# achinastone/Tensorium

Hardware: AMD Instinct MI355X
Metric: fp32 SGEMM GFLOP/s (M=N=K=4096) + YOLOv3 conv-fwd images/s (higher is better)
Workload: dtype fp32; 1 GPU; sgemm_nn_4096x4096x4096; M=4096, N=4096, K=4096, parallelism=1 independent replicas, one process per GPU, no data-path collective

## Files before the change

### tensorium_amd/csrc/conv_slab.hip

```cpp
#include <algorithm>
#include <type_traits>

#include "tns_act.hpp"
#include "tns_internal.hpp"

namespace tns {
namespace {

typedef float floatx4 __attribute__((ext_vector_type(4)));

__device__ __forceinline__ void slab_dma16(const float* sbase, unsigned voff, unsigned lds) {
  unsigned keep;
  asm volatile(
      "s_mov_b32 %0, m0\n\ts_mov_b32 m0, %3\n\ts_nop 0\n\t"
      "global_load_lds_dwordx4 %1, %2\n\ts_mov_b32 m0, %0"
      : "=&s"(keep)
      : "v"(voff), "s"(sbase), "s"(lds)
      : "memory");
}

struct SlabFillArgs {
  const float* x;
  int64_t strideX;
  float* slab;
  int C, H, W, stride, pad, dil, ow, ohw, N, K, KT;
  float inv_ohw, inv_ow;
  unsigned bytes;
  int64_t units;
};

__device__ __forceinline__ int slab_div(int n, int d, float inv) {
  int qq = (int)((float)n * inv);
  while (qq * d > n) --qq;
  while ((qq + 1) * d <= n) ++qq;
  return qq;
}

template <int KS, int BK, int BN>
__global__ __launch_bounds__(256) void slab_fill_kernel(SlabFillArgs a) {
  constexpr int NG = BK / 16, KK = KS * KS;
  const int64_t x = (int64_t)blockIdx.x * 256 + threadIdx.x;
  if (x >= a.units) return;
  const int c = (int)(x % BN);
  const int64_t r1 = x / BN;
  const int g = (int)(r1 % NG);
  const int64_t r2 = r1 / NG;
  const int t = (int)(r2 % a.KT), ct = (int)(r2 / a.KT);
  const int n = ct * BN + c;
  float v[16];
  const __amdgpu_buffer_rsrc_t rsrc =
      __builtin_amdgcn_make_buffer_rsrc(const_cast<float*>(a.x), 0, a.bytes, 0x00020000);
  {
    const int nn = n < a.N ? n : a.N - 1;
    const int img = slab_div(nn, a.ohw, a.inv_ohw), pix = nn - img * a.ohw;
    const int oy = slab_div(pix, a.ow, a.inv_ow), ox = pix - oy * a.ow;
    const int iy0 = oy * a.stride - a.pad, ix0 = ox * a.stride - a.pad;
    const int HW = a.H * a.W;
    unsigned mask = 0;
    int toff[KK];
#pragma unroll
    for (int kr = 0; kr < KS; ++kr)
#pragma unroll
      for (int kc = 0; kc < KS; ++kc) {
        const int iy = iy0 + kr * a.dil, ix = ix0 + kc * a.dil;
        mask |= (unsigned)(((unsigned)iy < (unsigned)a.H) & ((unsigned)ix < (unsigned)a.W))
                << (kr * KS + kc);
        toff[kr * KS + kc] = 4 * (kr * a.dil * a.W + kc * a.dil);
      }
    if (n >= a.N) mask = 0;
    const unsigned base = 4u * (unsigned)(img * (int)a.strideX + iy0 * a.W + ix0);
    const int k0 = t * BK + 16 * g;
    int ch = k0 / KK, tap = k0 - ch * KK;
#pragma unroll
    for (int e = 0; e < 16; ++e) {
      int off = toff[0];
#pragma unroll
      for (int u = 1; u < KK; ++u) off = tap == u ? toff[u] : off;
      const unsigned o = ((mask >> tap) & 1u) ? base + 4u * (unsigned)(ch * HW) + (unsigned)off
                                              : 0x80000000u;
      v[e] = __builtin_bit_cast(float, __builtin_amdgcn_raw_buffer_load_b32(rsrc, o, 0, 0));
      if (++tap == KK) {
        tap = 0;
        ++ch;
      }
    }
  }
  float* dst = a.slab + ((r2 * NG + g) * 4 * BN + c) * 4;
#pragma unroll
  for (int q = 0; q < 4; ++q)
    *reinterpret_cast<floatx4*>(dst + q * BN * 4) = floatx4{v[q], v[4 + q], v[8 + q], v[12 + q]};
}

template <int KS, int BK, int BN>
__global__ __launch_bounds__((BN + 63) / 64 * 64) void slab_fill_u_kernel(SlabFillArgs a) {
  constexpr int NG = BK / 16, KK = KS * KS;
  const int c = threadIdx.x;
  if (c >= BN) return;
  const int64_t r1 = blockIdx.x;
  const int g = (int)(r1 % NG);
  const int64_t r2 = r1 / NG;
  const int t = (int)(r2 % a.KT), ct = (int)(r2 / a.KT);
  const int n = ct * BN + c;
  float v[16];
  const __amdgpu_buffer_rsrc_t rsrc =
      __builtin_amdgcn_make_buffer_rsrc(const_cast<float*>(a.x), 0, a.bytes, 0x00020000);
  {
    const int nn = n < a.N ? n : a.N - 1;
    const int img = slab_div(nn, a.ohw, a.inv_ohw), pix = nn - img * a.ohw;
    const int oy = slab_div(pix, a.ow, a.inv_ow), ox = pix - oy * a.ow;
    const int iy0 = oy * a.stride - a.pad, ix0 = ox * a.stride - a.pad;
    const int HW = a.H * a.W;
    unsigned mask = 0;
#pragma unroll
    for (int kr = 0; kr < KS; ++kr)
#pragma unroll
      for (int kc = 0; kc < KS; ++kc) {
        const int iy = iy0 + kr * a.dil, ix = ix0 + kc * a.dil;
        mask |= (unsigned)(((unsigned)iy < (unsigned)a.H) & ((unsigned)ix < (unsigned)a.W))
                << (kr * KS + kc);
      }
    if (n >= a.N) mask = 0;
    const unsigned base = 4u * (unsigned)(img * (int)a.strideX + iy0 * a.W + ix0);
    const int k0 = __builtin_amdgcn_readfirstlane(t * BK + 16 * g);
    int ch = k0 / KK, tap = k0 - ch * KK;
    int kr = tap / KS, kc = tap - kr * KS;
#pragma unroll
    for (int e = 0; e < 16; ++e) {
      const unsigned uoff = 4u * (unsigned)(ch * HW + kr * a.dil * a.W + kc * a.dil);
      const unsigned o = ((mask >> tap) & 1u) ? base + uoff : 0x80000000u;
      v[e] = __builtin_bit_cast(float, __builtin_amdgcn_raw_buffer_load_b32(rsrc, o, 0, 0));
      ++tap;
      if (++kc == KS) {
        kc = 0;
        ++kr;
      }
      if (tap == KK) {
        tap = 0;
        kr = 0;
        ++ch;
      }
    }
  }
  float* dst = a.slab + ((r2 * NG + g) * 4 * BN + c) * 4;
#pragma unroll
  for (int q = 0; q < 4; ++q)
    *reinterpret_cast<floatx4*>(dst + q * BN * 4) = floatx4{v[q], v[4 + q], v[8 + q], v[12 + q]};
}

struct SlabGemmArgs {
  const float* A;
  const float* slab;
  float* C;
  const float* bias;
  int M, N, K, KT, tiles_m, ohw, act;
  bool fuse;
};

template <int BM_, int BN_, int BK_, int WM_, int WN_, int JA_, int NA_, int NS_, int DG_ = 0,
          int MAP_ = 0>
struct SG {
  static constexpr int BM = BM_, BN = BN_, BK = BK_, WM = WM_, WN = WN_, JA = JA_, NA = NA_;
  static constexpr int NS = NS_;
  static constexpr int DG = DG_, MAP = MAP_;
  static constexpr int NW = WM * WN, NT = 64 * NW, J = BN / 16, NG = BK / 16, ROWS = BK / 4;
  static constexpr int JB = NA < WN ? (J - NA * JA) / (WN - NA) : 0;
  static constexpr int A_TILE = ROWS * BM * 4, B_TILE = ROWS * BN * 4, STAGE = A_TILE + B_TILE;
  static constexpr int AU = BM * BK / 4 / NT;
  static constexpr int BDMA = 4 * BK * BN / 1024;
  static constexpr int DPW = (BDMA + NW - 1) / NW;
  static_assert(BM == 16 * WM && BN % 16 == 0 && BK % 16 == 0, "geometry");
  static_assert(NA * JA + (WN - NA) * JB == J && NA >= 1 && NA <= WN, "wave column split");
  static_assert(AU >= 1 && BM * BK / 4 % NT == 0, "A units");
  static_assert(4 * BK * BN % 1024 == 0, "whole DMA instructions");
  static_assert(NS >= 2 && NS * STAGE * 4 <= 163840, "LDS");
  static_assert(NG >= 2 && NG % 2 == 0, "groups: f0 holds group 0 at every tile start");
  static_assert(DPW * (NS - 2) <= 63 && DPW <= 63, "vmcnt immediates");
};

template <int JW>
struct SFrag {
  floatx4 a, b[JW];
};

template <int N>
__device__ __forceinline__ void wait_vm(bool keep_n) {
  if (keep_n)
    asm volatile("s_waitcnt vmcnt(%0)" ::"n"(N) : "memory");
  else
    asm volatile("s_waitcnt vmcnt(0)" ::: "memory");
}

template <class G>
__global__ __launch_bounds__(G::NT, 1) void slab_gemm_kernel(SlabGemmArgs p) {
  constexpr int BM = G::BM, BN = G::BN, BK = G::BK, NG = G::NG, NS = G::NS;
  constexpr int A_TILE = G::A_TILE, STAGE = G::STAGE, AU = G::AU, DPW = G::DPW;
  __shared__ __attribute__((aligned(16))) float smem[NS * STAGE];
  const int tid = threadIdx.x, lane = tid & 63;
  const int w = __builtin_amdgcn_readfirstlane(tid >> 6), wm = w % G::WM, wn = w / G::WM;
  const int r16 = lane & 15, q = lane >> 4;
  int tm, tn;
  {
    const int nb = gridDim.x, bid = blockIdx.x;
    const int xcd = bid & 7, qq = nb >> 3, rr = nb & 7;
    const int wg = (xcd < rr ? xcd * (qq + 1) : rr * (qq + 1) + (xcd - rr) * qq) + (bid >> 3);
    if constexpr (G::MAP == 1) {
      const int tiles_n = (p.N + BN - 1) / BN;
      tn = wg % tiles_n;
      tm = wg / tiles_n;
    } else {
      tm = wg % p.tiles_m;
      tn = wg / p.tiles_m;
    }
  }
  const int m0 = tm * BM, n0 = tn * BN;
  const int N = p.N, K = p.K, nt = p.KT;
  const float* slabT = p.slab + (int64_t)tn * K * BN;
  const unsigned lds0 = (unsigned)(uintptr_t)(__attribute__((address_space(3))) float*)smem;
  const unsigned voff = 16u * (unsigned)lane;
  auto dma_b = [&](int t, int st, int v) {
    if constexpr (G::DG & 1) return;
    int u = w + G::NW * v;
    if (G::BDMA % G::NW != 0 && u >= G::BDMA) u -= G::NW;
    slab_dma16(slabT + (int64_t)t * (BK * BN) + 256 * u, voff,
               lds0 + 4u * (unsigned)(st * STAGE + A_TILE) + 1024u * (unsigned)u);
  };
  auto dma_all = [&](int t, int st) {
#pragma unroll
    for (int v = 0; v < DPW; ++v) dma_b(t, st, v);
  };
  unsigned a_off[AU];
  int a_dst[AU];
#pragma unroll
  for (int u = 0; u < AU; ++u) {
    const int idx = tid + G::NT * u;
    const int lo = idx & 7, rest = idx >> 3;
    const int m = rest % BM, kq4 = lo + 8 * (rest / BM);
    a_off[u] = 4u * (unsigned)(m * K + 4 * kq4);
    a_dst[u] = (4 * (kq4 >> 2)) * BM * 4 + m * 4 + (kq4 & 3);
  }
  const float* a_row0 = p.A + (int64_t)m0 * K;
  floatx4 ra[AU];
  auto load_a = [&](int t) {
    if constexpr (G::DG & 2) return;
    const float* sb = a_row0 + t * BK;
#pragma unroll
    for (int u = 0; u < AU; ++u)
      asm volatile("global_load_dwordx4 %0, %1, %2" : "=v"(ra[u]) : "v"(a_off[u]), "s"(sb) : "memory");
  };
  auto store_a = [&](int st) {
    if constexpr (G::DG & 2) return;
    float* as = smem + st * STAGE;
#pragma unroll
    for (int u = 0; u < AU; ++u) {
      asm volatile("" : "+v"(ra[u]));
      as[a_dst[u]] = ra[u][0];
      as[a_dst[u] + BM * 4] = ra[u][1];
      as[a_dst[u] + 2 * BM * 4] = ra[u][2];
      as[a_dst[u] + 3 * BM * 4] = ra[u][3];
    }
  };

  auto run = [&](auto JWC, const int coff) {
    constexpr int JW = decltype(JWC)::value;
    floatx4 acc[JW];
#pragma unroll
    for (int j = 0; j < JW; ++j) acc[j] = floatx4{0.f, 0.f, 0.f, 0.f};
    using Frag = SFrag<JW>;
    auto frag = [&](int st, int g, Frag& f) {
      const float* ap = smem + st * STAGE + ((4 * g + q) * BM + wm * 16 + r16) * 4;
      f.a = *reinterpret_cast<const floatx4*>(ap);
      const float* bp = smem + st * STAGE + A_TILE + ((4 * g + q) * BN + coff * 16 + r16) * 4;
#pragma unroll
      for (int j = 0; j < JW; ++j) f.b[j] = *reinterpret_cast<const floatx4*>(bp + 64 * j);
    };
    auto mma = [&](const Frag& f) {
#pragma unroll
      for (int i = 0; i < 4; ++i)
#pragma unroll
        for (int j = 0; j < JW; ++j)
          acc[j] = __builtin_amdgcn_mfma_f32_16x16x4f32(f.a[i], f.b[j][i], acc[j], 0, 0, 0);
    };
    auto mma_dma = [&](const Frag& f, int tb, int st) {
      constexpr int NM = 4 * JW, STEP = NM / DPW > 0 ? NM / DPW : 1;
#pragma unroll
      for (int x = 0; x < NM; ++x) {
        const int i = x / JW, j = x % JW;
        acc[j] = __builtin_amdgcn_mfma_f32_16x16x4f32(f.a[i], f.b[j][i], acc[j], 0, 0, 0);
        if (x % STEP == 0 && x / STEP < DPW) dma_b(tb, st, x / STEP);
        __builtin_amdgcn_sched_barrier(0);
      }
      if constexpr (NM / STEP < DPW) {
#pragma unroll
        for (int v = NM / STEP; v < DPW; ++v) dma_b(tb, st, v);
      }
    };

    Frag f0, f1;
    load_a(0);
#pragma unroll
    for (int t = 0; t < NS; ++t) {
      if (t == 1 && nt > 1) {
        wait_vm<0>(false);
        store_a(0);
        load_a(1);
      }
      if (t < nt) dma_all(t, t);
    }
    if (nt == 1) {
      wait_vm<0>(false);
      store_a(0);
    } else {
      if (nt >= NS)
        asm volatile("s_waitcnt vmcnt(%0)" ::"n"(AU + (NS - 1) * DPW) : "memory");
      else
        wait_vm<0>(false);
    }
    __syncthreads();
    frag(0, 0, f0);
    for (int t = 0; t < nt; ++t) {
      const int cur = t % NS;
#pragma unroll
      for (int g = 0; g + 1 < NG; ++g) {
        Frag& fc = (g & 1) ? f1 : f0;
        Frag& fn = (g & 1) ? f0 : f1;
        frag(cur, g + 1, fn);
        __builtin_amdgcn_sched_barrier(0);
        mma(fc);
        __builtin_amdgcn_sched_barrier(0);
      }
      if (t + 1 < nt) {
        const int nxt = (t + 1) % NS;
        if constexpr (NS == 2)
          wait_vm<0>(false);
        else
          wait_vm<DPW>(t + NS - 1 < nt);
        store_a(nxt);
        if constexpr (!(G::DG & 4))
          __syncthreads();
        frag(nxt, 0, f0);
        if (t + 2 < nt) load_a(t + 2);
        __builtin_amdgcn_sched_barrier(0);
        if (t + NS < nt)
          mma_dma(f1, t + NS, cur);
        else
          mma(f1);
      } else {
        mma(f1);
      }
    }

    const int row0 = m0 + wm * 16 + 4 * q;
    float bias[4];
#pragma unroll
    for (int e = 0; e < 4; ++e) bias[e] = p.fuse ? p.bias[row0 + e] : 0.0f;
#pragma unroll
    for (int j = 0; j < JW; ++j) {
      const int n = n0 + coff * 16 + 16 * j + r16;
      if (n >= N) continue;
      const int img = n / p.ohw, pix = n - img * p.ohw;
      float* cp = p.C + ((int64_t)img * p.M + row0) * p.ohw + pix;
#pragma unroll
      for (int e = 0; e < 4; ++e) {
        float v = acc[j][e];
        if (p.fuse) v = act_apply_cheap(v + bias[e], p.act);
        cp[(int64_t)e * p.ohw] = v;
      }
    }
  };
  if constexpr (G::NA == G::WN) {
    run(std::integral_constant<int, G::JA>{}, wn * G::JA);
  } else {
    if (wn < G::NA)
      run(std::integral_constant<int, G::JA>{}, wn * G::JA);
    else
      run(std::integral_constant<int, G::JB>{}, G::NA * G::JA + (wn - G::NA) * G::JB);
  }
}

struct SlabForm {
  int bm, bn, bk;
  hipError_t (*gemm)(const SlabGemmArgs&, hipStream_t);
  hipError_t (*fill)(const SlabFillArgs&, int ks, hipStream_t);
  const char* name;
};

template <class G>
hipError_t launch_slab_gemm(const SlabGemmArgs& a, hipStream_t s) {
  const int64_t blocks = (int64_t)(a.M / G::BM) * ((a.N + G::BN - 1) / G::BN);
  hipLaunchKernelGGL((slab_gemm_kernel<G>), dim3((unsigned)blocks), dim3(G::NT), 0, s, a);
  return hipGetLastError();
}

template <int BK, int BN>
hipError_t launch_slab_fill(const SlabFillArgs& a, int ks, hipStream_t s) {
#ifndef TNS_SLAB_FILL_LANE
  {
    constexpr int NT = (BN + 63) / 64 * 64;
    const int64_t nb = a.units / BN;
    if (nb > 0x7fffffffLL) return hipErrorInvalidValue;
    if (ks == 3)
      hipLaunchKernelGGL((slab_fill_u_kernel<3, BK, BN>), dim3((unsigned)nb), dim3(NT), 0, s, a);
    else if (ks == 1)
      hipLaunchKernelGGL((slab_fill_u_kernel<1, BK, BN>), dim3((unsigned)nb), dim3(NT), 0, s, a);
    else
      return hipErrorInvalidValue;
    return hipGetLastError();
  }
#endif
  const unsigned blocks = (unsigned)((a.units + 255) / 256);
  if (ks == 3)
    hipLaunchKernelGGL((slab_fill_kernel<3, BK, BN>), dim3(blocks), dim3(256), 0, s, a);
  else if (ks == 1)
    hipLaunchKernelGGL((slab_fill_kernel<1, BK, BN>), dim3(blocks), dim3(256), 0, s, a);
  else
    return hipErrorInvalidValue;
  return hipGetLastError();
}

#define TNS_SLAB(BMv, BNv, BKv, WMv, WNv, JAv, NAv, NSv)                                       \
  {BMv, BNv, BKv, launch_slab_gemm<SG<BMv, BNv, BKv, WMv, WNv, JAv, NAv, NSv>>,                   \
   launch_slab_fill<BKv, BNv>,                                                                   \
   "conv_slab<" #BMv "x" #BNv "x" #BKv ",w" #WMv "x" #WNv ",j" #JAv "x" #NAv ",s" #NSv ">"}
#define TNS_SLABD(BMv, BNv, BKv, WMv, WNv, JAv, NAv, NSv, DGv, MAPv)                             \
  {BMv, BNv, BKv, launch_slab_gemm<SG<BMv, BNv, BKv, WMv, WNv, JAv, NAv, NSv, DGv, MAPv>>,       \
   launch_slab_fill<BKv, BNv>,                                                                   \
   "conv_slab<" #BMv "x" #BNv "x" #BKv ",w" #WMv "x" #WNv ",j" #JAv "x" #NAv ",s" #NSv ",dg" #DGv \
   ",map" #MAPv ">"}
const SlabForm kSlab[] = {
    TNS_SLAB(32, 176, 64, 2, 4, 3, 3, 3),
    TNS_SLAB(64, 176, 32, 4, 2, 6, 1, 3),
    TNS_SLAB(64, 176, 32, 4, 2, 6, 1, 4),
    TNS_SLAB(32, 176, 64, 2, 4, 3, 3, 2),
    TNS_SLAB(64, 176, 64, 4, 2, 6, 1, 2),
    TNS_SLAB(32, 176, 32, 2, 2, 6, 1, 4),
    TNS_SLABD(32, 176, 64, 2, 4, 3, 3, 2, 0, 1),
    TNS_SLABD(64, 176, 64, 4, 2, 6, 1, 2, 0, 1),
};
#undef TNS_SLAB
#undef TNS_SLABD
constexpr int kNumSlab = sizeof(kSlab) / sizeof(kSlab[0]);

}

int conv_slab_count() { return kNumSlab; }
const char* conv_slab_name(int v) { return v >= 0 && v < kNumSlab ? kSlab[v].name : ""; }

int conv_slab_pick(int64_t M, int64_t N, int64_t K, int64_t ks) {
  if (ks != 3 || K % 64) return -1;
  if (M == 1024 && N >= 1024) return 3;
  if (M == 512 && N >= 4096) return 4;
  return -1;
}

int64_t conv_slab_floats(int v, int64_t N, int64_t K) {
  if (v < 0 || v >= kNumSlab) return -1;
  const int64_t bn = kSlab[v].bn;
  return (N + bn - 1) / bn * bn * K;
}

hipError_t launch_conv_slab(int v, const ConvSlabArgs& c, float* slab, hipStream_t s) {
  if (v < 0 || v >= kNumSlab) return hipErrorInvalidValue;
  const SlabForm& f = kSlab[v];
  const int64_t N = c.batch * c.ohw;
  if (c.M % f.bm || c.K % f.bk || (c.ks != 1 && c.ks != 3) || N >= (1LL << 22) ||
      4 * c.batch * c.C * c.H * c.W > 0x7fffffffLL ||
      c.K > 0x7fffffffLL / f.bn || (reinterpret_cast<uintptr_t>(c.weights) & 15) || c.K % 4 ||
      (reinterpret_cast<uintptr_t>(slab) & 15) || c.M * c.K > 0x7fffffffLL)
    return hipErrorInvalidValue;
  const int64_t CT = (N + f.bn - 1) / f.bn, KT = c.K / f.bk;
  if (CT * (c.M / f.bm) > 0x7fffffffLL) return hipErrorInvalidValue;
  SlabFillArgs fa{};
  fa.x = c.input; fa.strideX = c.C * c.H * c.W; fa.slab = slab;
  fa.C = (int)c.C; fa.H = (int)c.H; fa.W = (int)c.W; fa.stride = (int)c.stride;
  fa.pad = (int)c.pad; fa.dil = (int)c.dil; fa.ow = (int)c.ow; fa.ohw = (int)c.ohw;
  fa.N = (int)N; fa.K = (int)c.K; fa.KT = (int)KT;
  fa.inv_ohw = (float)((1.0 + 1.0 / 1048576.0) / (double)c.ohw);
  fa.inv_ow = (float)((1.0 + 1.0 / 1048576.0) / (double)c.ow);
  fa.bytes = (unsigned)(4 * c.batch * c.C * c.H * c.W);
  fa.units = CT * KT * (f.bk / 16) * f.bn;
  if (hipError_t e = f.fill(fa, (int)c.ks, s)) return e;
  SlabGemmArgs ga{};
  ga.A = c.weights; ga.slab = slab; ga.C = c.out; ga.bias = c.bias;
  ga.M = (int)c.M; ga.N = (int)N; ga.K = (int)c.K; ga.KT = (int)KT;
  ga.tiles_m = (int)(c.M / f.bm); ga.ohw = (int)c.ohw; ga.act = c.act; ga.fuse = c.bias != nullptr;
  return f.gemm(ga, s);
}

}
```

Measured before the change: 148,800 GFLOP/s.

## Deepen A-operand register prefetch in slab conv GEMM pipeline

Adds an A-depth template parameter so the slab GEMM kernel keeps several tiles of A loads in flight in rotating register buffers, and waits with computed vmcnt immediates instead of a single-tile lookahead. The picked variants for the 1024- and 512-channel conv cases now use depths 2 and 4 to hide global-load latency on A with NS=2 LDS stages. It also removes the unused lane-parallel fill kernel. Deeper prefetch costs more VGPRs and a more complex prologue and wait accounting, which risks register pressure or mistimed waits. The SGEMM headline path is not touched.

Measured after the change: 148,800 GFLOP/s. No clear change (-0.0%).

```diff
diff --git a/tensorium_amd/csrc/conv_slab.hip b/tensorium_amd/csrc/conv_slab.hip
--- a/tensorium_amd/csrc/conv_slab.hip
+++ b/tensorium_amd/csrc/conv_slab.hip
@@ -34,61 +34,6 @@
   while (qq * d > n) --qq;
   while ((qq + 1) * d <= n) ++qq;
   return qq;
-}
-
-template <int KS, int BK, int BN>
-__global__ __launch_bounds__(256) void slab_fill_kernel(SlabFillArgs a) {
-  constexpr int NG = BK / 16, KK = KS * KS;
-  const int64_t x = (int64_t)blockIdx.x * 256 + threadIdx.x;
-  if (x >= a.units) return;
-  const int c = (int)(x % BN);
-  const int64_t r1 = x / BN;
-  const int g = (int)(r1 % NG);
-  const int64_t r2 = r1 / NG;
-  const int t = (int)(r2 % a.KT), ct = (int)(r2 / a.KT);
-  const int n = ct * BN + c;
-  float v[16];
-  const __amdgpu_buffer_rsrc_t rsrc =
-      __builtin_amdgcn_make_buffer_rsrc(const_cast<float*>(a.x), 0, a.bytes, 0x00020000);
-  {
-    const int nn = n < a.N ? n : a.N - 1;
-    const int img = slab_div(nn, a.ohw, a.inv_ohw), pix = nn - img * a.ohw;
-    const int oy = slab_div(pix, a.ow, a.inv_ow), ox = pix - oy * a.ow;
-    const int iy0 = oy * a.stride - a.pad, ix0 = ox * a.stride - a.pad;
-    const int HW = a.H * a.W;
-    unsigned mask = 0;
-    int toff[KK];
-#pragma unroll
-    for (int kr = 0; kr < KS; ++kr)
-#pragma unroll
-      for (int kc = 0; kc < KS; ++kc) {
-        const int iy = iy0 + kr * a.dil, ix = ix0 + kc * a.dil;
-        mask |= (unsigned)(((unsigned)iy < (unsigned)a.H) & ((unsigned)ix < (unsigned)a.W))
-                << (kr * KS + kc);
-        toff[kr * KS + kc] = 4 * (kr * a.dil * a.W + kc * a.dil);
-      }
-    if (n >= a.N) mask = 0;
-    const unsigned base = 4u * (unsigned)(img * (int)a.strideX + iy0 * a.W + ix0);
-    const int k0 = t * BK + 16 * g;
-    int ch = k0 / KK, tap = k0 - ch * KK;
-#pragma unroll
-    for (int e = 0; e < 16; ++e) {
-      int off = toff[0];
-#pragma unroll
-      for (int u = 1; u < KK; ++u) off = tap == u ? toff[u] : off;
-      const unsigned o = ((mask >> tap) & 1u) ? base + 4u * (unsigned)(ch * HW) + (unsigned)off
-                                              : 0x80000000u;
-      v[e] = __builtin_bit_cast(float, __builtin_amdgcn_raw_buffer_load_b32(rsrc, o, 0, 0));
-      if (++tap == KK) {
-        tap = 0;
-        ++ch;
-      }
-    }
-  }
-  float* dst = a.slab + ((r2 * NG + g) * 4 * BN + c) * 4;
-#pragma unroll
-  for (int q = 0; q < 4; ++q)
-    *reinterpret_cast<floatx4*>(dst + q * BN * 4) = floatx4{v[q], v[4 + q], v[8 + q], v[12 + q]};
 }
 
 template <int KS, int BK, int BN>
@@ -157,11 +102,12 @@
 };
 
 template <int BM_, int BN_, int BK_, int WM_, int WN_, int JA_, int NA_, int NS_, int DG_ = 0,
-          int MAP_ = 0>
+          int MAP_ = 0, int AD_ = 1>
 struct SG {
   static constexpr int BM = BM_, BN = BN_, BK = BK_, WM = WM_, WN = WN_, JA = JA_, NA = NA_;
   static constexpr int NS = NS_;
   static constexpr int DG = DG_, MAP = MAP_;
+  static constexpr int AD = AD_;
   static constexpr int NW = WM * WN, NT = 64 * NW, J = BN / 16, NG = BK / 16, ROWS = BK / 4;
   static constexpr int JB = NA < WN ? (J - NA * JA) / (WN - NA) : 0;
   static constexpr int A_TILE = ROWS * BM * 4, B_TILE = ROWS * BN * 4, STAGE = A_TILE + B_TILE;
@@ -175,6 +121,10 @@
   static_assert(NS >= 2 && NS * STAGE * 4 <= 163840, "LDS");
   static_assert(NG >= 2 && NG % 2 == 0, "groups: f0 holds group 0 at every tile start");
   static_assert(DPW * (NS - 2) <= 63 && DPW <= 63, "vmcnt immediates");
+  static constexpr int KEEP_A = (AD < NS ? AD : NS) - 1;
+  static constexpr int KEEP_B = AD - 1 < NS - 2 ? AD - 1 : NS - 2;
+  static constexpr int KEEP = AU * KEEP_A + DPW * KEEP_B;
+  static_assert(AD >= 1 && AD <= 4 && (AD == 1 || KEEP <= 63), "A depth");
 };
 
 template <int JW>
@@ -239,24 +189,28 @@
     a_dst[u] = (4 * (kq4 >> 2)) * BM * 4 + m * 4 + (kq4 & 3);
   }
   const float* a_row0 = p.A + (int64_t)m0 * K;
-  floatx4 ra[AU];
-  auto load_a = [&](int t) {
+  constexpr int AD = G::AD;
+  floatx4 ra[AD][AU];
+  auto load_a = [&](int t, floatx4(&r)[AU]) __attribute__((always_inline)) {
     if constexpr (G::DG & 2) return;
     const float* sb = a_row0 + t * BK;
 #pragma unroll
     for (int u = 0; u < AU; ++u)
-      asm volatile("global_load_dwordx4 %0, %1, %2" : "=v"(ra[u]) : "v"(a_off[u]), "s"(sb) : "memory");
+      asm volatile("global_load_dwordx4 %0, %1, %2"
+                   : "=v"(r[u])
+                   : "v"(a_off[u]), "s"(sb)
+                   : "memory");
   };
-  auto store_a = [&](int st) {
+  auto store_a = [&](int st, floatx4(&r)[AU]) __attribute__((always_inline)) {
     if constexpr (G::DG & 2) return;
     float* as = smem + st * STAGE;
 #pragma unroll
     for (int u = 0; u < AU; ++u) {
-      asm volatile("" : "+v"(ra[u]));
-      as[a_dst[u]] = ra[u][0];
-      as[a_dst[u] + BM * 4] = ra[u][1];
-      as[a_dst[u] + 2 * BM * 4] = ra[u][2];
-      as[a_dst[u] + 3 * BM * 4] = ra[u][3];
+      asm volatile("" : "+v"(r[u]));
+      as[a_dst[u]] = r[u][0];
+      as[a_dst[u] + BM * 4] = r[u][1];
+      as[a_dst[u] + 2 * BM * 4] = r[u][2];
+      as[a_dst[u] + 3 * BM * 4] = r[u][3];
     }
   };
 
@@ -296,56 +250,117 @@
     };
 
     Frag f0, f1;
-    load_a(0);
-#pragma unroll
-    for (int t = 0; t < NS; ++t) {
-      if (t == 1 && nt > 1) {
+    if constexpr (AD == 1) {
+      load_a(0, ra[0]);
+#pragma unroll
+      for (int t = 0; t < NS; ++t) {
+        if (t == 1 && nt > 1) {
+          wait_vm<0>(false);
+          store_a(0, ra[0]);
+          load_a(1, ra[0]);
+        }
+        if (t < nt) dma_all(t, t);
+      }
+      if (nt == 1) {
         wait_vm<0>(false);
-        store_a(0);
-        load_a(1);
-      }
-      if (t < nt) dma_all(t, t);
-    }
-    if (nt == 1) {
-      wait_vm<0>(false);
-      store_a(0);
+        store_a(0, ra[0]);
+      } else {
+        if (nt >= NS)
+          asm volatile("s_waitcnt vmcnt(%0)" ::"n"(AU + (NS - 1) * DPW) : "memory");
+        else
+          wait_vm<0>(false);
+      }
+      __syncthreads();
+      frag(0, 0, f0);
+      for (int t = 0; t < nt; ++t) {
+        const int cur = t % NS;
+#pragma unroll
+        for (int g = 0; g + 1 < NG; ++g) {
+          Frag& fc = (g & 1) ? f1 : f0;
+          Frag& fn = (g & 1) ? f0 : f1;
+          frag(cur, g + 1, fn);
+          __builtin_amdgcn_sched_barrier(0);
+          mma(fc);
+          __builtin_amdgcn_sched_barrier(0);
+        }
+        if (t + 1 < nt) {
+          const int nxt = (t + 1) % NS;
+          if constexpr (NS == 2)
+            wait_vm<0>(false);
+          else
+            wait_vm<DPW>(t + NS - 1 < nt);
+          store_a(nxt, ra[0]);
+          if constexpr (!(G::DG & 4))
+            __syncthreads();
+          frag(nxt, 0, f0);
+          if (t + 2 < nt) load_a(t + 2, ra[0]);
+          __builtin_amdgcn_sched_barrier(0);
+          if (t + NS < nt)
+            mma_dma(f1, t + NS, cur);
+          else
+            mma(f1);
+        } else {
+          mma(f1);
+        }
+      }
     } else {
-      if (nt >= NS)
-        asm volatile("s_waitcnt vmcnt(%0)" ::"n"(AU + (NS - 1) * DPW) : "memory");
-      else
-        wait_vm<0>(false);
-    }
-    __syncthreads();
-    frag(0, 0, f0);
-    for (int t = 0; t < nt; ++t) {
-      const int cur = t % NS;
-#pragma unroll
-      for (int g = 0; g + 1 < NG; ++g) {
-        Frag& fc = (g & 1) ? f1 : f0;
-        Frag& fn = (g & 1) ? f0 : f1;
-        frag(cur, g + 1, fn);
-        __builtin_amdgcn_sched_barrier(0);
-        mma(fc);
-        __builtin_amdgcn_sched_barrier(0);
-      }
-      if (t + 1 < nt) {
-        const int nxt = (t + 1) % NS;
-        if constexpr (NS == 2)
-          wait_vm<0>(false);
-        else
-          wait_vm<DPW>(t + NS - 1 < nt);
-        store_a(nxt);
-        if constexpr (!(G::DG & 4))
-          __syncthreads();
-        frag(nxt, 0, f0);
-        if (t + 2 < nt) load_a(t + 2);
-        __builtin_amdgcn_sched_barrier(0);
-        if (t + NS < nt)
-          mma_dma(f1, t + NS, cur);
-        else
+      constexpr int LAG = AD > NS - 1 ? AD : NS - 1;
+      auto slot_dma = [&](int tb) __attribute__((always_inline)) {
+        if (tb >= 0 && tb < nt) dma_all(tb, tb % NS);
+      };
+      constexpr int SL = AD + 1 > NS ? AD + 1 : NS;
+#pragma unroll
+      for (int s = -SL; s <= -2; ++s) {
+        slot_dma(s + NS);
+        const int ta = s + AD + 1;
+        if (ta >= 0 && ta < nt) {
+          if (ta % AD == 0) load_a(ta, ra[0]);
+          if constexpr (AD > 1) if (ta % AD == 1) load_a(ta, ra[1 % AD]);
+          if constexpr (AD > 2) if (ta % AD == 2) load_a(ta, ra[2 % AD]);
+          if constexpr (AD > 3) if (ta % AD == 3) load_a(ta, ra[3 % AD]);
+        }
+      }
+      wait_vm<G::KEEP>(LAG - 1 < nt);
+      store_a(0, ra[0]);
+      __syncthreads();
+      frag(0, 0, f0);
+      slot_dma(NS - 1);
+      if (AD < nt) load_a(AD, ra[0]);
+      auto tile = [&](int t, auto UC) __attribute__((always_inline)) {
+        constexpr int NX = (decltype(UC)::value + 1) % AD;
+        const int cur = t % NS;
+#pragma unroll
+        for (int g = 0; g + 1 < NG; ++g) {
+          Frag& fc = (g & 1) ? f1 : f0;
+          Frag& fn = (g & 1) ? f0 : f1;
+          frag(cur, g + 1, fn);
+          __builtin_amdgcn_sched_barrier(0);
+          mma(fc);
+          __builtin_amdgcn_sched_barrier(0);
+        }
+        if (t + 1 < nt) {
+          const int nxt = (t + 1) % NS;
+          wait_vm<G::KEEP>(t + LAG < nt);
+          store_a(nxt, ra[NX]);
+          if constexpr (!(G::DG & 4))
+            __syncthreads();
+          frag(nxt, 0, f0);
+          __builtin_amdgcn_sched_barrier(0);
+          if (t + NS < nt)
+            mma_dma(f1, t + NS, cur);
+          else
+            mma(f1);
+          __builtin_amdgcn_sched_barrier(0);
+          if (t + AD + 1 < nt) load_a(t + AD + 1, ra[NX]);
+        } else {
           mma(f1);
-      } else {
-        mma(f1);
+        }
+      };
+      for (int t0 = 0; t0 < nt; t0 += AD) {
+        tile(t0, std::integral_constant<int, 0>{});
+        if constexpr (AD > 1) if (t0 + 1 < nt) tile(t0 + 1, std::integral_constant<int, 1 % AD>{});
+        if constexpr (AD > 2) if (t0 + 2 < nt) tile(t0 + 2, std::integral_constant<int, 2 % AD>{});
+        if constexpr (AD > 3) if (t0 + 3 < nt) tile(t0 + 3, std::integral_constant<int, 3 % AD>{});
       }
     }
 
@@ -393,51 +408,44 @@
 
 template <int BK, int BN>
 hipError_t launch_slab_fill(const SlabFillArgs& a, int ks, hipStream_t s) {
-#ifndef TNS_SLAB_FILL_LANE
-  {
-    constexpr int NT = (BN + 63) / 64 * 64;
-    const int64_t nb = a.units / BN;
-    if (nb > 0x7fffffffLL) return hipErrorInvalidValue;
-    if (ks == 3)
-      hipLaunchKernelGGL((slab_fill_u_kernel<3, BK, BN>), dim3((unsigned)nb), dim3(NT), 0, s, a);
-    else if (ks == 1)
-      hipLaunchKernelGGL((slab_fill_u_kernel<1, BK, BN>), dim3((unsigned)nb), dim3(NT), 0, s, a);
-    else
-      return hipErrorInvalidValue;
-    return hipGetLastError();
-  }
-#endif
-  const unsigned blocks = (unsigned)((a.units + 255) / 256);
+  constexpr int NT = (BN + 63) / 64 * 64;
+  const int64_t nb = a.units / BN;
+  if (nb > 0x7fffffffLL) return hipErrorInvalidValue;
   if (ks == 3)
-    hipLaunchKernelGGL((slab_fill_kernel<3, BK, BN>), dim3(blocks), dim3(256), 0, s, a);
+    hipLaunchKernelGGL((slab_fill_u_kernel<3, BK, BN>), dim3((unsigned)nb), dim3(NT), 0, s, a);
   else if (ks == 1)
-    hipLaunchKernelGGL((slab_fill_kernel<1, BK, BN>), dim3(blocks), dim3(256), 0, s, a);
+    hipLaunchKernelGGL((slab_fill_u_kernel<1, BK, BN>), dim3((unsigned)nb), dim3(NT), 0, s, a);
   else
     return hipErrorInvalidValue;
   return hipGetLastError();
 }
 
-#define TNS_SLAB(BMv, BNv, BKv, WMv, WNv, JAv, NAv, NSv)                                       \
-  {BMv, BNv, BKv, launch_slab_gemm<SG<BMv, BNv, BKv, WMv, WNv, JAv, NAv, NSv>>,                   \
+#define TNS_SLABX(BMv, BNv, BKv, WMv, WNv, JAv, NAv, NSv, DGv, MAPv, ADv, TAIL)                  \
+  {BMv, BNv, BKv, launch_slab_gemm<SG<BMv, BNv, BKv, WMv, WNv, JAv, NAv, NSv, DGv, MAPv, ADv>>,  \
    launch_slab_fill<BKv, BNv>,                                                                   \
-   "conv_slab<" #BMv "x" #BNv "x" #BKv ",w" #WMv "x" #WNv ",j" #JAv "x" #NAv ",s" #NSv ">"}
-#define TNS_SLABD(BMv, BNv, BKv, WMv, WNv, JAv, NAv, NSv, DGv, MAPv)                             \
-  {BMv, BNv, BKv, launch_slab_gemm<SG<BMv, BNv, BKv, WMv, WNv, JAv, NAv, NSv, DGv, MAPv>>,       \
-   launch_slab_fill<BKv, BNv>,                                                                   \
-   "conv_slab<" #BMv "x" #BNv "x" #BKv ",w" #WMv "x" #WNv ",j" #JAv "x" #NAv ",s" #NSv ",dg" #DGv \
-   ",map" #MAPv ">"}
+   "conv_slab<" #BMv "x" #BNv "x" #BKv ",w" #WMv "x" #WNv ",j" #JAv "x" #NAv ",s" #NSv TAIL ">"}
+#define TNS_SLAB(BMv, BNv, BKv, WMv, WNv, JAv, NAv, NSv, ADv) \
+  TNS_SLABX(BMv, BNv, BKv, WMv, WNv, JAv, NAv, NSv, 0, 0, ADv, "")
+#define TNS_SLABD(BMv, BNv, BKv, WMv, WNv, JAv, NAv, NSv, DGv, MAPv) \
+  TNS_SLABX(BMv, BNv, BKv, WMv, WNv, JAv, NAv, NSv, DGv, MAPv, 1, ",dg" #DGv ",map" #MAPv)
+#define TNS_SLABA(BMv, BNv, BKv, WMv, WNv, JAv, NAv, NSv, ADv) \
+  TNS_SLABX(BMv, BNv, BKv, WMv, WNv, JAv, NAv, NSv, 0, 0, ADv, ",a" #ADv)
 const SlabForm kSlab[] = {
-    TNS_SLAB(32, 176, 64, 2, 4, 3, 3, 3),
-    TNS_SLAB(64, 176, 32, 4, 2, 6, 1, 3),
-    TNS_SLAB(64, 176, 32, 4, 2, 6, 1, 4),
-    TNS_SLAB(32, 176, 64, 2, 4, 3, 3, 2),
-    TNS_SLAB(64, 176, 64, 4, 2, 6, 1, 2),
-    TNS_SLAB(32, 176, 32, 2, 2, 6, 1, 4),
+    TNS_SLAB(32, 176, 64, 2, 4, 3, 3, 3, 1),
+    TNS_SLAB(64, 176, 32, 4, 2, 6, 1, 3, 1),
+    TNS_SLAB(64, 176, 32, 4, 2, 6, 1, 4, 1),
+    TNS_SLAB(32, 176, 64, 2, 4, 3, 3, 2, 2),
+    TNS_SLAB(64, 176, 64, 4, 2, 6, 1, 2, 4),
+    TNS_SLAB(32, 176, 32, 2, 2, 6, 1, 4, 1),
     TNS_SLABD(32, 176, 64, 2, 4, 3, 3, 2, 0, 1),
     TNS_SLABD(64, 176, 64, 4, 2, 6, 1, 2, 0, 1),
+    TNS_SLABA(32, 176, 64, 2, 4, 3, 3, 2, 1),
+    TNS_SLABA(64, 176, 64, 4, 2, 6, 1, 2, 1),
 };
 #undef TNS_SLAB
 #undef TNS_SLABD
+#undef TNS_SLABA
+#undef TNS_SLABX
 constexpr int kNumSlab = sizeof(kSlab) / sizeof(kSlab[0]);
 
 }
```
